# bergmanlab/TELR

Measured on AMD Instinct MI355X. Metric: gbp_aligned_per_s, higher is better.
Workload: dtype int16

## Files before the change

telr_amd/csrc/kernels.hip.h:

```cpp
#pragma once
#include <hip/hip_runtime.h>
#include <stdint.h>

#define TELR_NEG      (-(1 << 28))
#include "part_plan.h"
#define SK_TILE       1024
#define SK_THREADS    256
#define DP_DMAX       4096

struct ChainOpt {
    int32_t max_gap, bw, min_cnt, min_chain_score, chain_gap_q8, chain_skip_q8;
    int32_t dense_n, dense_span, mw_n;
};
struct DpOpt {
    int32_t a, b, q, e, q2, e2, sc_ambi, zdrop;
    int32_t cx_scale, cx_open, cx_emax, cx_emin, cx_dec, cx_flat;
};
__host__ __device__ __forceinline__ int d_cx_ext(const DpOpt &o, int len) { int v = o.cx_emax - o.cx_dec * len; return v > o.cx_emin ? v : o.cx_emin; }
__host__ __device__ __forceinline__ int d_cx_cost(const DpOpt &o, int L)
{
    int t = o.cx_open;
    for (int i = 0; i < L && i < o.cx_flat; ++i) t += d_cx_ext(o, i);
    if (L > o.cx_flat) t += (L - o.cx_flat) * o.cx_emin;
    return t;
// ... 3219 lines not shown
                const int delta = mx < -8192 ? 0 : mx;
                const uint32_t dd = pk_dup(delta), thr = pk_dup(delta - 12000);
#define REB_ONE(x) { const uint32_t dead = pk_sign(pk_sub((x), thr)); (x) = pk_sel(dead, PK_NEG, pk_max(pk_sub((x), dd), PK_NEG)); }
#pragma unroll
                for (int r = 0; r < R; ++r) { REB_ONE(He[r]) REB_ONE(Ho[r]) REB_ONE(E1e[r]) REB_ONE(E1o[r]) REB_ONE(F1e[r]) REB_ONE(F1o[r]) }
#undef REB_ONE
                off += delta;
            }
        }
        if (NW > 1) {
            if (wl == 63) { uint32_t *x = xch + (1 * NW + wv) * 3; x[0] = Ho[R - 1]; x[1] = E1o[R - 1]; x[2] = E2o[R - 1]; }
            __syncthreads();
        }
        if (EXT && __all(done)) break;
    }
    if (EXT) {
        if (have && l == 0) {
            DpRes Rr; Rr.score = best; Rr.bi = bi; Rr.bj = bj; Rr.nops = 0; Rr.mlen = 0; Rr.cells = ncell; Rr.tbases = n; Rr.mcols = 0;
            A.res[prob] = Rr;
        }
        return;
    }
    if (fin_here) {
        int sc = (int)(short)(fin_hi ? (fin >> 16) : (fin & 0xffffu)) + fin_off;
        if constexpr (TB4) sc >>= 2;
        if constexpr (TAG8) sc >>= 3;
        DpRes Rr; Rr.score = sc; Rr.bi = m; Rr.bj = n; Rr.nops = 0; Rr.mlen = 0; Rr.cells = P.pad[1]; Rr.tbases = n; Rr.mcols = 0;
        A.res[prob] = Rr;
    }
}

#define PK_NC 9
static_assert(__builtin_popcount(CLSM_PK) == PK_NC, "PK_NC counts the DPF_PK rows of DP_CLASS");
__host__ __device__ __forceinline__ constexpr int PK_IDX(int cls) { return __builtin_popcount(CLSM_PK & ((1u << cls) - 1u)); }
__host__ __device__ __forceinline__ constexpr int PK_CLS(int c) { int cls = 0; for (int k = 0; k < DP_NCLS; ++k) if (d_cls_in(k, CLSM_PK) && PK_IDX(k) == c) cls = k; return cls; }
struct PkPlan { int32_t woff[PK_NC + 1]; };
__global__ void k_pk_waves(const DpProb *__restrict__ probs, const int32_t *__restrict__ cls_list, ClsOff off, PkPlan plan,
                           uint32_t *__restrict__ keys, uint32_t *__restrict__ vals)
{
    const int i = blockIdx.x * blockDim.x + threadIdx.x;
    if (i >= plan.woff[PK_NC]) return;
    int c = 0;
    while (i >= plan.woff[c + 1]) ++c;
    const int cls = PK_CLS(c), first = (i - plan.woff[c]) * (64 / DP_CLASS[cls].lpp);
    const DpProb P = probs[cls_list[off.off[cls] + first]];
    const uint32_t cost = (uint32_t)((P.m + P.n) * DP_CLASS[cls].regs);
    keys[i] = cost > 0xFFFFu ? 0xFFFFu : cost;
    vals[i] = (uint32_t)cls << 26 | (uint32_t)first;
}
enum PkCell : int { CELL_PLAIN, CELL_TAG8, CELL_CX, CELL_ONEP, CELL_NIBBLE };
__device__ __forceinline__ int d_pk_cell(int cls, const DpOpt &o, int tb4, int tag8_steps, const DpProb *__restrict__ probs, const int32_t *__restrict__ first)
{
    if (o.cx_scale) return CELL_CX;
    const int onep_d = d_onep_d(o.q, o.e, o.q2, o.e2);
    static_assert(DP_CLASS[CLS_PK16].nibble == 1 && DP_CLASS[CLS_PK20].nibble == 2, "the nibble classes and their tb4_mask bits");
    if ((cls == CLS_PK16 && onep_d >= DP_CLASS[CLS_PK16].maxd) || (cls == CLS_PK20 && onep_d >= DP_CLASS[CLS_PK20].maxd)) return d_tb4(cls, tb4) ? CELL_NIBBLE : CELL_ONEP;
    const DpProb P0 = probs[*first];
    return P0.m + P0.n <= tag8_steps ? CELL_TAG8 : CELL_PLAIN;
}
template <int CLS, bool EXACT, bool ONEP, bool TB4, bool TAG8, bool CX>
__device__ __forceinline__ void d_dp_pk_cls(const DpArgs &A, const int32_t *__restrict__ list, int n, int first)
{
    static_assert(DP_CLASS[CLS].family == DPF_PK && EXACT == (DP_CLASS[CLS].layout == TBL_INTERLEAVED && CLS != CLS_PK16), "class table");
    d_dp_pkr<DP_CLASS[CLS].lpp, DP_CLASS[CLS].regs, false, 1, EXACT ? DP_CLASS[CLS].regs - 1 : 0, ONEP, TB4, TAG8, CX>(A, list, n, first);
}
template <bool TAG8, bool CX>
__device__ __forceinline__ void d_dp_pk_any(int cls, const DpArgs &A, const int32_t *__restrict__ list, int n, int first)
{
    switch (cls) {
    case CLS_PK20: d_dp_pk_cls<CLS_PK20, true, false, false, TAG8, CX>(A, list, n, first); break;
    case CLS_PK24: d_dp_pk_cls<CLS_PK24, true, false, false, TAG8, CX>(A, list, n, first); break;
    case CLS_PK28: d_dp_pk_cls<CLS_PK28, true, false, false, TAG8, CX>(A, list, n, first); break;
    case CLS_PK32: d_dp_pk_cls<CLS_PK32, true, false, false, TAG8, CX>(A, list, n, first); break;
    case CLS_PK16: d_dp_pk_cls<CLS_PK16, false, false, false, TAG8, CX>(A, list, n, first); break;
    case CLS_PK40: d_dp_pk_cls<CLS_PK40, false, false, false, TAG8, CX>(A, list, n, first); break;
    case CLS_PK48: d_dp_pk_cls<CLS_PK48, false, false, false, TAG8, CX>(A, list, n, first); break;
    case CLS_PK128: d_dp_pk_cls<CLS_PK128, false, false, false, TAG8, CX>(A, list, n, first); break;
    default: d_dp_pk_cls<CLS_PK64, false, false, false, TAG8, CX>(A, list, n, first); break;
    }
}
#ifndef PK_WPE
#define PK_WPE 2
#endif
__global__ void __launch_bounds__(64) __attribute__((amdgpu_waves_per_eu(PK_WPE))) k_dp_pk(DpArgs A, const uint32_t *__restrict__ waves, const int32_t *__restrict__ cls_list,
                                              ClsOff off)
{
    const uint32_t w = waves[blockIdx.x];
    const int cls = (int)(w >> 26), first = (int)(w & 0x3ffffffu);
    const int32_t *list = cls_list + off.off[cls];
    const int n = off.off[cls + 1] - off.off[cls];
    const int cell = d_pk_cell(cls, A.o, A.tb4, A.tag8_steps, A.probs, list + first);
    if (cell == CELL_CX) { d_dp_pk_any<false, true>(cls, A, list, n, first); return; }
    if (cell >= CELL_ONEP && cls == CLS_PK16) { if (cell == CELL_NIBBLE) d_dp_pk_cls<CLS_PK16, false, true, true, false, false>(A, list, n, first); else d_dp_pk_cls<CLS_PK16, false, true, false, false, false>(A, list, n, first); return; }
    if (cell >= CELL_ONEP) { if (cell == CELL_NIBBLE) d_dp_pk_cls<CLS_PK20, true, true, true, false, false>(A, list, n, first); else d_dp_pk_cls<CLS_PK20, true, true, false, false, false>(A, list, n, first); return; }
    if (cell == CELL_TAG8) { d_dp_pk_any<true, false>(cls, A, list, n, first); return; }
    d_dp_pk_any<false, false>(cls, A, list, n, first);
}
template <int NW>
__global__ void __launch_bounds__(64 * NW) k_dp_pkw(DpArgs A)
{
    __shared__ uint32_t xch[2 * NW * 3 + NW];
    __builtin_amdgcn_s_setprio(3);
    if (A.o.cx_scale) d_dp_pkr<64 * NW, 1, false, NW, 0, false, false, false, true>(A, A.list, A.nlist, blockIdx.x, xch);
    else d_dp_pkr<64 * NW, 1, false, NW>(A, A.list, A.nlist, blockIdx.x, xch);
}
constexpr int PKX_LPP = DP_CLASS[CLS_PKX64].lpp, PKX_R = DP_CLASS[CLS_PKX64].regs;
__global__ void __launch_bounds__(64) k_dp_pkx(DpArgs A)
{
    __builtin_amdgcn_s_setprio(3);
    if (A.o.cx_scale) d_dp_pkr<PKX_LPP, PKX_R, true, 1, 0, false, false, false, true>(A, A.list, A.nlist, blockIdx.x * (64 / PKX_LPP));
    else d_dp_pkr<PKX_LPP, PKX_R, true>(A, A.list, A.nlist, blockIdx.x * (64 / PKX_LPP));
}
__global__ void __launch_bounds__(64) k_dp_pkx16(DpArgs A)
{
    __builtin_amdgcn_s_setprio(3);
    if (A.o.cx_scale) d_dp_pkr<16, 1, true, 1, 0, false, false, false, true>(A, A.list, A.nlist, blockIdx.x * 4);
    else d_dp_pkr<16, 1, true>(A, A.list, A.nlist, blockIdx.x * 4);
}

constexpr int PKX8_LPP = DP_CLASS[CLS_PKX128].lpp;
static_assert(DP_CLASS[CLS_PKX128].regs == 32 / PKX8_LPP && DP_CLASS[CLS_PKX256].lpp == 16 && DP_CLASS[CLS_PKX256].regs == 4, "class table");
__global__ void __launch_bounds__(64) k_dp_pkx_w8(DpArgs A)
{
    __builtin_amdgcn_s_setprio(3);
    if (A.o.cx_scale) d_dp_pkr<PKX8_LPP, 32 / PKX8_LPP, true, 1, 0, false, false, false, true>(A, A.list, A.nlist, blockIdx.x * (64 / PKX8_LPP));
    else d_dp_pkr<PKX8_LPP, 32 / PKX8_LPP, true>(A, A.list, A.nlist, blockIdx.x * (64 / PKX8_LPP));
}
__global__ void __launch_bounds__(64) k_dp_pkx_w16(DpArgs A)
{
    __builtin_amdgcn_s_setprio(3);
    if (A.o.cx_scale) d_dp_pkr<16, 4, true, 1, 0, false, false, false, true>(A, A.list, A.nlist, blockIdx.x * 4);
    else d_dp_pkr<16, 4, true>(A, A.list, A.nlist, blockIdx.x * 4);
}

#ifndef TB_SLOTS
#define TB_SLOTS 2
#endif
template <int LAYOUT>
__device__ __forceinline__ void d_traceback_lane(const DpProb *__restrict__ probs, DpRes *__restrict__ res, int pi,
                                                 const uint8_t *__restrict__ tb_all, uint32_t *__restrict__ cig, int32_t *__restrict__ retry,
                                                 uint32_t *stage)
{
    const int lane = threadIdx.x;
    const DpProb P = probs[pi];
    if (P.kind >= 3) return;
    const int dhi_ = P.dhi; int touched = 0;
    const int cls = P.pad[0] & 0xff, dlo = P.dlo, mg = P.pad[0] >> 8;
    const int D = P.dhi - dlo + 1, stride = (D + 2) / 2;
    const int lpp = d_cls_slots(cls);
    const bool packed = d_tb_regs(cls), tiled = d_tb_tiled(cls), rows2 = d_tb_rows2(cls);
    int i = res[pi].bi, j = res[pi].bj;
    uint32_t *cg = cig + P.cig_off;
    int no = 0, ml = 0, mc = 0, state = 0, cur_op = -1, cur_len = 0;
    const int rowb = tiled ? lpp * 16 : packed ? lpp * 4 : stride;
    int64_t tag0 = -1, tag1 = -1, pfb = -2;
    uint4 v0 = make_uint4(0, 0, 0, 0), v1 = v0, v2 = v0, v3 = v0, v4 = v0, v5 = v0, v6 = v0, v7 = v0;
    while (i > 0 && j > 0) {
        const int a = i + j, sl = (j - i - dlo) >> 1;
        const int64_t off = tiled ? ((((int64_t)(a >> 3) * (4 * lpp) + ((sl >> 3) << 4) + (((a >> 1) & 3) << 2) + ((sl >> 1) & 3)) << 2) + ((a & 1) << 1) + (sl & 1))
                          : (LAYOUT == 2 || rows2) ? ((((int64_t)(a >> 1) * lpp + (sl >> 1)) << 2) + ((a & 1) << 1) + (sl & 1))
                          : packed ? ((((int64_t)(a >> 2) * lpp + sl) << 2) + (a & 3)) : ((int64_t)a * stride + sl);
        const int64_t abs_off = P.tb_off + (d_tb_interleaved(cls) ? ((off >> 3) << 9) + (off & 7) : off), line = abs_off >> 6;
        const int slot = TB_SLOTS > 1 ? (int)(line & 1) : 0;
        if ((slot ? tag1 : tag0) != line) {
            const int64_t blk = line >> 1;
            if (pfb != blk) {
                const uint4 *src = (const uint4*)(tb_all + (blk << 7));
                v0 = src[0]; v1 = src[1]; v2 = src[2]; v3 = src[3]; v4 = src[4]; v5 = src[5]; v6 = src[6]; v7 = src[7];
            }
            uint32_t *dst = stage + slot * 1024 + lane;
            if (line & 1) {
                dst[0 * 64] = v4.x; dst[1 * 64] = v4.y; dst[2 * 64] = v4.z; dst[3 * 64] = v4.w;
                dst[4 * 64] = v5.x; dst[5 * 64] = v5.y; dst[6 * 64] = v5.z; dst[7 * 64] = v5.w;
                dst[8 * 64] = v6.x; dst[9 * 64] = v6.y; dst[10 * 64] = v6.z; dst[11 * 64] = v6.w;
                dst[12 * 64] = v7.x; dst[13 * 64] = v7.y; dst[14 * 64] = v7.z; dst[15 * 64] = v7.w;
            } else {
                dst[0 * 64] = v0.x; dst[1 * 64] = v0.y; dst[2 * 64] = v0.z; dst[3 * 64] = v0.w;
                dst[4 * 64] = v1.x; dst[5 * 64] = v1.y; dst[6 * 64] = v1.z; dst[7 * 64] = v1.w;
                dst[8 * 64] = v2.x; dst[9 * 64] = v2.y; dst[10 * 64] = v2.z; dst[11 * 64] = v2.w;
                dst[12 * 64] = v3.x; dst[13 * 64] = v3.y; dst[14 * 64] = v3.z; dst[15 * 64] = v3.w;
            }
            if (slot) tag1 = line; else tag0 = line;
            const int64_t nl = rowb >= 64 ? (abs_off - rowb) >> 6 : line - 1, nb = nl >> 1;
            pfb = blk;
            if (nb != blk && nl >= 0) {
                const uint4 *src = (const uint4*)(tb_all + (nb << 7));
                v0 = src[0]; v1 = src[1]; v2 = src[2]; v3 = src[3]; v4 = src[4]; v5 = src[5]; v6 = src[6]; v7 = src[7];
                pfb = nb;
            }
        }
        const int w = (int)(abs_off & 63);
        const uint8_t *st8 = (const uint8_t*)stage + ((slot * 1024 + lane) << 2);
        const uint32_t t = st8[(w >> 2) * 256 + (w & 3)];
        const int mij = i < j ? i : j, kr = tiled ? (a >> 1) & 3 : 0;
        const bool up1 = kr >= 1 && mij > 1, up2 = kr >= 2 && mij > 2, up3 = kr >= 3 && mij > 3;
        const uint32_t t1 = up1 ? st8[((w - 16) >> 2) * 256 + (w & 3)] : 0xffu, t2 = up2 ? st8[((w - 32) >> 2) * 256 + (w & 3)] : 0xffu, t3 = up3 ? st8[((w - 48) >> 2) * 256 + (w & 3)] : 0xffu;
        const uint32_t nd = (uint32_t)((t1 & 7u) != 0u) << 1 | (uint32_t)((t2 & 7u) != 0u) << 2 | (uint32_t)((t3 & 7u) != 0u) << 3;
        const uint32_t mb = (t >> 7) | ((t1 >> 7) & 1u) << 1 | ((t2 >> 7) & 1u) << 2 | ((t3 >> 7) & 1u) << 3;
        touched |= (j - i - dlo <= mg) | (dhi_ - (j - i) <= mg);
        const int s0 = state ? state : (int)(t & 7);
        const int isM = s0 == 0, isD = s0 & 1;
        const int op = isM ? 0 : (isD ? 2 : 1);
        const int nn = isM ? __builtin_ctz(nd | 16u) : 1;
        state = (isM || !((t >> (2 + s0)) & 1)) ? 0 : s0;
        ml += isM ? __builtin_popcount(mb & ((1u << nn) - 1u)) : 0; mc += isM ? nn : 0;
        i -= isM ? nn : (isD ^ 1); j -= isM ? nn : isD;
        const bool same = op == cur_op;
        if (!same && cur_len) cg[no++] = (uint32_t)cur_len << 4 | (uint32_t)cur_op;
        cur_len = same ? cur_len + nn : nn; cur_op = op;
    }
    if (i > 0) { if (cur_op == 1) cur_len += i; else { if (cur_len) cg[no++] = (uint32_t)cur_len << 4 | (uint32_t)cur_op; cur_op = 1; cur_len = i; } }
    if (j > 0) { if (cur_op == 2) cur_len += j; else { if (cur_len) cg[no++] = (uint32_t)cur_len << 4 | (uint32_t)cur_op; cur_op = 2; cur_len = j; } }
    if (cur_len) cg[no++] = (uint32_t)cur_len << 4 | (uint32_t)cur_op;
    res[pi].nops = no; res[pi].mlen = ml; res[pi].mcols = mc;
    if (retry && P.kind == 0 && touched && P.m + P.n <= ADAPT_MAX_STEPS) retry[pi] = 1;
}
__global__ void __launch_bounds__(64) k_traceback(const DpProb *__restrict__ probs, DpRes *__restrict__ res, int32_t np,
                                                  const uint8_t *__restrict__ tb_all, uint32_t *__restrict__ cig, int32_t *__restrict__ retry,
                                                  const int32_t *__restrict__ list)
{
// ... 35 lines not shown
                x0 = make_uint4(u0.x, u0.y, u1.x, u1.y); x1 = make_uint4(u2.x, u2.y, u3.x, u3.y); x2 = make_uint4(u4.x, u4.y, u5.x, u5.y); x3 = make_uint4(u6.x, u6.y, u7.x, u7.y); } \
            else { const uint4 *src = (const uint4*)(tb + ((int64_t)L__ << 6)); x0 = src[0]; x1 = src[1]; x2 = src[2]; x3 = src[3]; } } } while (0)
#define TBR_PUT(dst_, x0, x1, x2, x3) do { uint32_t *dst = (dst_); \
            dst[0 * 64] = x0.x; dst[1 * 64] = x0.y; dst[2 * 64] = x0.z; dst[3 * 64] = x0.w; dst[4 * 64] = x1.x; dst[5 * 64] = x1.y; dst[6 * 64] = x1.z; dst[7 * 64] = x1.w; \
            dst[8 * 64] = x2.x; dst[9 * 64] = x2.y; dst[10 * 64] = x2.z; dst[11 * 64] = x2.w; dst[12 * 64] = x3.x; dst[13 * 64] = x3.y; dst[14 * 64] = x3.z; dst[15 * 64] = x3.w; } while (0)
#define TBR_ENSURE(L_) do { const int Le = (L_); \
            if (Le & 1) { if (tag1 != Le) { TBR_PUT(stage + 1024 + lane, b0, b1, b2, b3); tag1 = Le; TBR_FETCH(Le - 2, b0, b1, b2, b3); } } \
            else        { if (tag0 != Le) { TBR_PUT(stage + lane, a0, a1, a2, a3); tag0 = Le; TBR_FETCH(Le - 2, a0, a1, a2, a3); } } } while (0)
        if (ltop & 1) { TBR_FETCH(ltop, b0, b1, b2, b3); TBR_FETCH(ltop - 1, a0, a1, a2, a3); }
        else { TBR_FETCH(ltop, a0, a1, a2, a3); TBR_FETCH(ltop - 1, b0, b1, b2, b3); }
        for (int L = ltop; L >= 0; --L) {
            TBR_ENSURE(L);
            const int lim = L << 6;
            for (;;) {
                const int a = i + j, sl = (j - i - dlo) >> 1;
                const int o = nib ? (a >> 1) * rb4 + ((sl >> 2) << 2) + (((sl >> 1) & 1) << 1) + (sl & 1)
                                  : (((a >> 1) * lpp + (sl >> 1)) << 2) + ((a & 1) << 1) + (sl & 1);
                const bool act = i > 0 && j > 0 && o >= lim;
                if (!__any(act)) break;
                const int oo = act ? o : 0;
#define TBR_BYTE(x) ((uint32_t)stage8[((((x) >> 6) & 1) * 1024 + (((x) & 63) >> 2) * 64 + lane) * 4 + ((x) & 3)])
                const uint8_t *stage8 = (const uint8_t*)stage;
                uint32_t t = TBR_BYTE(oo);
                const int mij = i < j ? i : j, room = o - lim;
                const bool v1 = act && mij > 1 && room >= rowb, v2 = act && mij > 2 && room >= 2 * rowb, v3 = act && mij > 3 && room >= 3 * rowb;
                const uint32_t t1 = TBR_BYTE(v1 ? oo - rowb : 0), t2 = TBR_BYTE(v2 ? oo - 2 * rowb : 0), t3 = TBR_BYTE(v3 ? oo - 3 * rowb : 0);
#undef TBR_BYTE
                uint32_t nd, mb;
                if constexpr (ENC == 2) {
                    const int sh = (a & 1) << 2;
                    nd = (uint32_t)(!v1 || ((t1 >> sh) & 3u) != 2u) << 1 | (uint32_t)(!v2 || ((t2 >> sh) & 3u) != 2u) << 2 | (uint32_t)(!v3 || ((t3 >> sh) & 3u) != 2u) << 3;
                    mb = 0;
                    const uint32_t nb = (t >> sh) & 0xfu;
                    t = (2u - (nb & 3u)) | (nb & 4u) | ((nb & 8u) ^ 8u);
                } else if constexpr (ENC == 1) {
                    nd = (uint32_t)(!v1 || (t1 & 7u) != 4u) << 1 | (uint32_t)(!v2 || (t2 & 7u) != 4u) << 2 | (uint32_t)(!v3 || (t3 & 7u) != 4u) << 3;
                    mb = 0;
                    t = (4u - (t & 7u)) | (t & 0x28u) | ((t & 0x50u) ^ 0x50u);
                } else {
                    nd = (uint32_t)(!v1 || (t1 & 7u) != 0u) << 1 | (uint32_t)(!v2 || (t2 & 7u) != 0u) << 2 | (uint32_t)(!v3 || (t3 & 7u) != 0u) << 3;
                    mb = (t >> 7) | (t1 >> 7) << 1 | (t2 >> 7) << 2 | (t3 >> 7) << 3;
                }
                if (act) {
                    touched |= (j - i - dlo <= mg) | (dhi_ - (j - i) <= mg);
                    const int s0 = state ? state : (int)(t & (nib ? 3 : 7));
                    const int isM = s0 == 0, isD = s0 & 1;
                    const int op = isM ? 0 : (isD ? 2 : 1);
                    const int nn = isM ? __builtin_ctz(nd | 16u) : 1;
                    if (!isM) gc += (s0 <= 2 ? o_.e : o_.e2) + (state ? 0 : (s0 <= 2 ? o_.q : o_.q2));
                    state = (isM || !((t >> ((nib ? 1 : 2) + s0)) & 1)) ? 0 : s0;
                    ml += isM ? __builtin_popcount(mb & ((1u << nn) - 1u)) : 0; mc += isM ? nn : 0;
                    i -= isM ? nn : (isD ^ 1); j -= isM ? nn : isD;
                    const bool same = op == cur_op;
                    if (!same && cur_len) cg[no++] = (uint32_t)cur_len << 4 | (uint32_t)cur_op;
                    cur_len = same ? cur_len + nn : nn; cur_op = op;
                }
            }
            if (!__any(i > 0 && j > 0)) break;
        }
#undef TBR_FETCH
#undef TBR_PUT
#undef TBR_ENSURE
    }
    if (!have) return;
    if (i > 0) { const int c1 = o_.q + o_.e * i, c2 = o_.q2 + o_.e2 * i; gc += c1 < c2 ? c1 : c2; }
    if (j > 0) { const int c1 = o_.q + o_.e * j, c2 = o_.q2 + o_.e2 * j; gc += c1 < c2 ? c1 : c2; }
    if (i > 0) { if (cur_op == 1) cur_len += i; else { if (cur_len) cg[no++] = (uint32_t)cur_len << 4 | (uint32_t)cur_op; cur_op = 1; cur_len = i; } }
    if (j > 0) { if (cur_op == 2) cur_len += j; else { if (cur_len) cg[no++] = (uint32_t)cur_len << 4 | (uint32_t)cur_op; cur_op = 2; cur_len = j; } }
    if (cur_len) cg[no++] = (uint32_t)cur_len << 4 | (uint32_t)cur_op;
    if (nib || tag8) ml = (res[pi].score + o_.b * mc + gc) / (o_.a + o_.b);
    res[pi].nops = no; res[pi].mlen = ml; res[pi].mcols = mc;
    if (retry && P.kind == 0 && touched && P.m + P.n <= ADAPT_MAX_STEPS) retry[pi] = 1;
}
#ifdef TB_PROF
__device__ unsigned long long g_tb_prof[8];
#endif
__global__ void __launch_bounds__(64) k_traceback_pk(const DpProb *__restrict__ probs, DpRes *__restrict__ res,
                                                     const uint8_t *__restrict__ tb_all, uint32_t *__restrict__ cig, int32_t *__restrict__ retry,
                                                     const uint32_t *__restrict__ waves, const int32_t *__restrict__ cls_list, ClsOff off, int32_t tb4, DpOpt o, int32_t tag8_steps)
{
    __shared__ uint32_t stage[TB_SLOTS * 16 * 64];
    const uint32_t w = waves[blockIdx.x];
    const int cls = (int)(w >> 26), first = (int)(w & 0x3ffffffu);
    const int ppw = 64 / DP_CLASS[cls].lpp, t = threadIdx.x;
    const bool have = t < ppw && first + t < off.off[cls + 1] - off.off[cls];
    const int cell = d_pk_cell(cls, o, tb4, tag8_steps, probs, cls_list + off.off[cls] + first), rb4 = cell == CELL_NIBBLE ? d_tb4_rowb(cls) : 0;
    const bool tag8 = cell == CELL_TAG8;
#ifdef TB_PROF
    const unsigned long long t0_ = wall_clock64();
#endif
    const int pi_ = cls_list[off.off[cls] + (have ? first + t : first)], lpp_ = d_cls_slots(cls);
    if (d_tb_interleaved(cls)) {
        if (rb4) d_traceback_rows<2, true>(probs, res, pi_, have, lpp_, rb4, o, tb_all, cig, retry, stage);
        else if (tag8) d_traceback_rows<1, true>(probs, res, pi_, have, lpp_, 0, o, tb_all, cig, retry, stage);
        else d_traceback_rows<0, true>(probs, res, pi_, have, lpp_, 0, o, tb_all, cig, retry, stage);
    } else if (tag8) d_traceback_rows<1, false>(probs, res, pi_, have, lpp_, 0, o, tb_all, cig, retry, stage);
    else d_traceback_rows<0, false>(probs, res, pi_, have, lpp_, 0, o, tb_all, cig, retry, stage);
#ifdef TB_PROF
    if (threadIdx.x == 0) {
        const unsigned long long t1_ = wall_clock64(), dt = t1_ - t0_;
        const int rowb_ = rb4 ? rb4 : d_cls_slots(cls) * 4;
        const DpProb P0 = probs[cls_list[off.off[cls] + first]];
        unsigned long long lines = (unsigned long long)(((P0.m + P0.n) / 2 + 1) * rowb_ + 63) >> 6; if (lines > 65535) lines = 65535;
        atomicAdd(&g_tb_prof[0], dt); atomicMax(&g_tb_prof[1], dt << 16 | lines); atomicAdd(&g_tb_prof[2], 1ULL); atomicAdd(&g_tb_prof[3], lines);
        atomicMin(&g_tb_prof[4], t0_); atomicMax(&g_tb_prof[5], t1_);
    }
#endif
}

__global__ void __launch_bounds__(64) k_traceback_w(const DpProb *__restrict__ probs, DpRes *__restrict__ res, int32_t np,
                                                    const uint8_t *__restrict__ tb_all, uint32_t *__restrict__ cig, int32_t *__restrict__ retry,
                                                    const int32_t *__restrict__ list)
{
    __shared__ uint32_t win[64 * 16];
    const int lane = threadIdx.x;
    if ((int)blockIdx.x >= np) return;
    const int pi = list ? list[blockIdx.x] : (int)blockIdx.x;
    const DpProb P = probs[pi];
    if (P.kind >= 3) return;
    const int dhi_ = P.dhi; int touched = 0;
    const int cls = P.pad[0] & 0xff, dlo = P.dlo, mg = P.pad[0] >> 8;
    const int D = P.dhi - dlo + 1, stride = (D + 2) / 2;
    const int lpp = d_cls_slots(cls);
    const bool packed = d_tb_regs(cls), rows2 = d_tb_rows2(cls);
    const int64_t rowb = packed ? (int64_t)lpp * 4 : stride;
    const uint8_t *tb = tb_all + P.tb_off;
    int i = res[pi].bi, j = res[pi].bj;
    uint32_t *cg = cig + P.cig_off;
    int no = 0, ml = 0, mc = 0, state = 0, cur_op = -1, cur_len = 0;
    int r0 = -1; int64_t c0 = 0;
    while (i > 0 && j > 0) {
        const int a = i + j, sl = (j - i - dlo) >> 1;
        int row; int64_t col;
        if (rows2) { row = a >> 1; col = ((int64_t)(sl >> 1) << 2) + ((a & 1) << 1) + (sl & 1); }
        else if (packed) { row = a >> 2; col = ((int64_t)sl << 2) + (a & 3); }
        else { row = a; col = sl; }
        const int k = r0 - row;
        if (r0 < 0 || k < 0 || k >= 64 || col < c0 || col >= c0 + 64) {
            __syncthreads();
            r0 = row; c0 = col - 32; if (c0 < 0) c0 = 0; c0 &= ~3LL;
            const int rk = r0 - lane;
            uint32_t v[16];
#pragma unroll
            for (int x = 0; x < 16; ++x) v[x] = 0;
            if (rk >= 0) {
                const int64_t byte0 = (int64_t)rk * rowb + c0;
                const uint32_t *src = (const uint32_t*)(tb + (byte0 & ~3LL));
                const int sh = (int)(byte0 & 3) * 8;
                if (sh == 0) {
#pragma unroll
                    for (int x = 0; x < 16; ++x) v[x] = src[x];
                } else {
                    uint32_t prev = src[0];
#pragma unroll
                    for (int x = 0; x < 16; ++x) { const uint32_t nx = src[x + 1]; v[x] = (prev >> sh) | (nx << (32 - sh)); prev = nx; }
                }
            }
#pragma unroll
            for (int x = 0; x < 16; ++x) win[lane * 16 + x] = v[x];
            __syncthreads();
        }
        const int w = (int)(col - c0);
        touched |= (j - i - dlo <= mg) | (dhi_ - (j - i) <= mg);
        if (state == 0) {
            const int ik = i - lane, jk = j - lane, ak = a - 2 * lane;
            int rowk; int64_t colk;
            if (rows2) { rowk = ak >> 1; colk = ((int64_t)(sl >> 1) << 2) + ((ak & 1) << 1) + (sl & 1); }
            else if (packed) { rowk = ak >> 2; colk = ((int64_t)sl << 2) + (ak & 3); }
            else { rowk = ak; colk = sl; }
            const int kk = r0 - rowk, wk = (int)(colk - c0);
            const bool inw = ik > 0 && jk > 0 && kk < 64 && wk >= 0 && wk < 64;
            const uint32_t tk = inw ? (win[kk * 16 + (wk >> 2)] >> ((wk & 3) * 8)) & 0xffu : 0xffu;
            const uint64_t stop = ~__ballot(inw && (tk & 7u) == 0u);
            const int run = stop ? __builtin_ctzll(stop) : 64;
            if (run > 0) {
                const uint64_t low = run >= 64 ? ~0ULL : (1ULL << run) - 1;
                ml += __builtin_popcountll(__ballot(inw && (tk >> 7)) & low); mc += run; i -= run; j -= run;
                if (cur_op == 0) cur_len += run;
                else { if (cur_len && lane == 0) cg[no] = (uint32_t)cur_len << 4 | (uint32_t)cur_op; if (cur_len) ++no; cur_op = 0; cur_len = run; }
                continue;
// ... 203 lines not shown
```

telr_amd/csrc/telr_engine.hip:

```cpp
#include <hip/hip_runtime.h>
#include <cstring>
#include <string.h>
#include <rocprim/rocprim.hpp>
#include <algorithm>
#include <atomic>
#include <immintrin.h>
#include <chrono>
#include <cmath>
#include <condition_variable>
#include <cstdio>
#include <cstdlib>
#include <cstring>
#include <map>
#include <memory>
#include <mutex>
#include <string>
#include <thread>
#include <sys/mman.h>
#include <vector>
#include "../../include/telr_hip.h"
#include "kernels.hip.h"
#include "range_plan.h"
#include "sam_records.h"
#define TELR_HAVE_SEED_ARGS 1
// ... 1337 lines not shown
        HIPCHK(rocprim::radix_sort_pairs(tmp, tbytes, d_clskey, d_keytmp, d_listtmp, d_clslist, (size_t)np, 0, 24, st));
    }
    if (np > 0) {
        int64_t *d_tbs;
        TRY(ctx_buf_t(ctx, ("tb_sorted" + sfx).c_str(), (size_t)np + 1, &d_tbs));
        hipLaunchKernelGGL(k_tb_gather, dim3(np / 256 + 1), dim3(256), 0, st, d_tbb, d_clslist, np, coff, d_tbs);
        TRY((dev_exclusive_scan<int64_t, int64_t>(ctx, d_tbs, d_tboff, (size_t)np + 1)));
        hipLaunchKernelGGL(k_tb_scatter, dim3(np / 256 + 1), dim3(256), 0, st, d_probs, d_clslist, np, coff, d_tboff);
        HIPCHK(hipGetLastError());
        HIPCHK(hipMemcpyAsync(&tb_total, d_tboff + np, 8, hipMemcpyDeviceToHost, st));
        HIPCHK(hipStreamSynchronize(st));
    }
    uint8_t *d_tb;
    TRY(ctx_buf_t(ctx, ("tb" + sfx).c_str(), (size_t)tb_total + 256, &d_tb));
    if (primary) TRY(ctx_buf_t(ctx, "rawcig", (size_t)cg_total + 16, d_rawcig_io));
    DpArgs D; D.qseq2 = qs->d_seq2; D.qnmask = qs->d_nmask; D.tseq2 = tg->d_seq2; D.tnmask = tg->d_nmask; D.probs = d_probs;
    D.qtot = qs->padded_bases; D.ttot = tg->padded_bases;
    D.o.a = mo->a; D.o.b = mo->b; D.o.q = mo->q; D.o.e = mo->e; D.o.q2 = mo->q2; D.o.e2 = mo->e2; D.o.sc_ambi = mo->sc_ambi; D.o.zdrop = mo->zdrop;
    D.o.cx_scale = D.o.cx_open = D.o.cx_emax = D.o.cx_emin = D.o.cx_dec = D.o.cx_flat = 0;
    if (mo->cx_scale > 0) {
        const int S = mo->cx_scale;
        D.o.a *= S; D.o.b *= S; D.o.sc_ambi *= S; D.o.zdrop *= S;
        D.o.cx_scale = S; D.o.cx_open = mo->cx_open; D.o.cx_emax = mo->cx_ext_max; D.o.cx_emin = mo->cx_ext_min; D.o.cx_dec = mo->cx_decay;
        D.o.cx_flat = mo->cx_decay > 0 && mo->cx_ext_max > mo->cx_ext_min ? (mo->cx_ext_max - mo->cx_ext_min + mo->cx_decay - 1) / mo->cx_decay : 0;
    }
    D.tb = d_tb; D.cig = *d_rawcig_io; D.res = d_res; D.dcap = 0;
    D.retry = d_retry; D.tb4 = L.tb4_mask; D.tag8_steps = L.tag8_steps;
    static const bool tb_split = !ab_on("tb_one_launch");
    int nw = 0; uint32_t *d_wv2 = nullptr;
    {
        PkPlan plan; plan.woff[0] = 0;
        for (int c = 0; c < PK_NC; ++c) { const int ppw = 64 / DP_CLASS[PK_CLS(c)].lpp; plan.woff[c + 1] = plan.woff[c] + (h_cls[PK_CLS(c)] + ppw - 1) / ppw; }
        nw = plan.woff[PK_NC];
        if (nw > 0) {
            uint32_t *d_wk, *d_wv, *d_wk2;
            TRY(ctx_buf_t(ctx, ("pk_wkey" + sfx).c_str(), (size_t)nw, &d_wk));
            TRY(ctx_buf_t(ctx, ("pk_wval" + sfx).c_str(), (size_t)nw, &d_wv));
            TRY(ctx_buf_t(ctx, ("pk_wkey2" + sfx).c_str(), (size_t)nw, &d_wk2));
            TRY(ctx_buf_t(ctx, ("pk_wval2" + sfx).c_str(), (size_t)nw, &d_wv2));
            hipLaunchKernelGGL(k_pk_waves, dim3((nw + 255) / 256), dim3(256), 0, st, d_probs, d_clslist, coff, plan, d_wk, d_wv);
            HIPCHK(hipGetLastError());
            size_t tbytes = 0;
            HIPCHK(rocprim::radix_sort_pairs_desc(nullptr, tbytes, d_wk, d_wk2, d_wv, d_wv2, (size_t)nw, 0, 16, st));
            void *tmp; TRY(ctx_buf(ctx, "rp_tmp", tbytes, &tmp));
            HIPCHK(rocprim::radix_sort_pairs_desc(tmp, tbytes, d_wk, d_wk2, d_wv, d_wv2, (size_t)nw, 0, 16, st));
        }
    }
    HIPCHK(hipEventRecord(ctx->ev_fork, st));
    int side = 0;
    std::vector<hipStream_t> used;
    static const bool serial = getenv("TELR_SERIAL") != nullptr;
    auto side_stream = [&]() { if (serial) return st; hipStream_t s2 = ctx->side[side % TELR_NSIDE]; ++side; used.push_back(s2); return s2; };
    auto launch = [&](int c, DpKernel kernel, hipStream_t s2) -> int {
        const int nl = h_cls[c];
        int threads = DP_CLASS[c].lpp > 64 ? DP_CLASS[c].lpp : 64, ppb = DP_CLASS[c].lpp < 64 ? 64 / DP_CLASS[c].lpp : 1;
        size_t lds = 0;
        D.list = d_clslist + coff.off[c]; D.nlist = nl; D.dcap = 0;
        if (DP_CLASS[c].family == DPF_LDS) {
            D.dcap = DP_CLASS[c].maxd;
            lds = (size_t)(D.dcap + 2) * 5 * 4;
            static const bool one_wave = ab_on("dp_one_wave");
            if (one_wave) { kernel = k_dp; threads = 64; }
            if (lds > 48 * 1024) HIPCHK(hipFuncSetAttribute((const void*)kernel, hipFuncAttributeMaxDynamicSharedMemorySize, (int)lds));
        }
        if (c == CLS_PKX64 && nl < 8192) { kernel = k_dp_pkx16; ppb = 4; }
        hipLaunchKernelGGL(kernel, dim3((nl + ppb - 1) / ppb), dim3(threads), lds, s2, D);
        HIPCHK(hipGetLastError());
        return TELR_OK;
    };
    for (const SideLaunch &row : SIDE_LAUNCH) {
        const int c = row.cls, nl = h_cls[c];
        if (nl == 0) continue;
        hipStream_t s2 = side_stream();
        HIPCHK(hipStreamWaitEvent(s2, ctx->ev_fork, 0));
        TRY(launch(c, row.kernel, s2));
        if (tb_split) {
            const int tbw_max = 2048;
            if (row.lane_walk || nl > tbw_max) hipLaunchKernelGGL(k_traceback, dim3((nl + 63) / 64), dim3(64), 0, s2, d_probs, d_res, nl, d_tb, *d_rawcig_io, d_retry, D.list);
            else hipLaunchKernelGGL(k_traceback_w, dim3(nl), dim3(64), 0, s2, d_probs, d_res, nl, d_tb, *d_rawcig_io, d_retry, D.list);
            HIPCHK(hipGetLastError());
        }
    }
    D.dcap = 0;
    const bool tb_over = tb_split && !serial && nw > 0;
    if (primary) HIPCHK(hipEventRecord(ctx->evk[5], st));
    if (primary && nw > 0) ++ctx->pk_launches;
    if (nw > 0) {
        D.list = nullptr; D.nlist = 0;
        if (tb_over) { HIPCHK(hipStreamWaitEvent(ctx->tb_stream, ctx->ev_fork, 0)); if (primary) HIPCHK(hipEventRecord(ctx->evk[3], ctx->tb_stream)); }
        hipLaunchKernelGGL(k_dp_pk, dim3(nw), dim3(64), 0, st, D, d_wv2, d_clslist, coff);
        HIPCHK(hipGetLastError());
        if (tb_over) {
            HIPCHK(hipEventRecord(ctx->ev_pk, st));
            HIPCHK(hipStreamWaitEvent(ctx->tb_stream, ctx->ev_pk, 0));
            hipLaunchKernelGGL(k_traceback_pk, dim3(nw), dim3(64), 0, ctx->tb_stream, d_probs, d_res, d_tb, *d_rawcig_io, d_retry, d_wv2, d_clslist, coff, L.tb4_mask, D.o, L.tag8_steps);
            HIPCHK(hipGetLastError());
            if (primary) HIPCHK(hipEventRecord(ctx->evk[4], ctx->tb_stream));
            used.push_back(ctx->tb_stream);
        }
    }
    if (primary) HIPCHK(hipEventRecord(ctx->evk[0], st));
    if (h_cls[CLS_REG64]) TRY(launch(CLS_REG64, reg_kernel<CLS_REG64>(), st));
    if (h_cls[CLS_REG128]) TRY(launch(CLS_REG128, reg_kernel<CLS_REG128>(), st));
    if (primary) HIPCHK(hipEventRecord(ctx->evk[1], st));
    if (tb_split) {
        if (!tb_over && primary) HIPCHK(hipEventRecord(ctx->evk[3], st));
        if (!tb_over && nw > 0) hipLaunchKernelGGL(k_traceback_pk, dim3(nw), dim3(64), 0, st, d_probs, d_res, d_tb, *d_rawcig_io, d_retry, d_wv2, d_clslist, coff, L.tb4_mask, D.o, L.tag8_steps);
        for (int c : { (int)CLS_REG128, (int)CLS_REG64 }) {
            if (h_cls[c] == 0) continue;
            hipLaunchKernelGGL(k_traceback, dim3((h_cls[c] + 63) / 64), dim3(64), 0, st, d_probs, d_res, h_cls[c], d_tb, *d_rawcig_io, d_retry, (const int32_t*)(d_clslist + coff.off[c]));
        }
        if (!tb_over && primary) HIPCHK(hipEventRecord(ctx->evk[4], st));
        HIPCHK(hipGetLastError());
    }
    for (size_t u = 0; u < used.size(); ++u) {
        HIPCHK(hipEventRecord(ctx->ev_side[u % TELR_NSIDE], used[u]));
        HIPCHK(hipStreamWaitEvent(st, ctx->ev_side[u % TELR_NSIDE], 0));
    }
#ifdef TB_PROF
    if (nw > 0) {
        HIPCHK(hipDeviceSynchronize());
        unsigned long long h[8]; HIPCHK(hipMemcpyFromSymbol(h, HIP_SYMBOL(g_tb_prof), sizeof(h)));
        unsigned long long z[8] = {0, 0, 0, 0, ~0ULL, 0, 0, 0}; HIPCHK(hipMemcpyToSymbol(HIP_SYMBOL(g_tb_prof), z, sizeof(z)));
        if (h[2]) fprintf(stderr, "[tb prof] k_traceback_pk: %llu waves, span %.3f ms, longest wave %.3f ms (%llu lines), mean wave %.3f ms, %.1f lines per wave, wave-ms / span = %.1f waves on the device on average\n",
                          h[2], (double)(h[5] - h[4]) / 1e5, (double)(h[1] >> 16) / 1e5, h[1] & 0xffffULL, (double)h[0] / (double)h[2] / 1e5, (double)h[3] / (double)h[2], (double)h[0] / (double)(h[5] - h[4] ? h[5] - h[4] : 1));
    }
#endif
    if (!tb_split) {
        if (primary) HIPCHK(hipEventRecord(ctx->evk[3], st));
        hipLaunchKernelGGL(k_traceback, dim3((np + 63) / 64), dim3(64), 0, st, d_probs, d_res, np, d_tb, *d_rawcig_io, d_retry, (const int32_t*)nullptr);
        if (primary) HIPCHK(hipEventRecord(ctx->evk[4], st));
    }
    HIPCHK(hipGetLastError());
    return TELR_OK;
}

struct HostTrace {
    bool on; const char *tag; std::chrono::steady_clock::time_point t0, last;
    HostTrace(const char *t) : tag(t) { static const bool e = trace_on("host"); on = e; t0 = last = std::chrono::steady_clock::now(); }
    void mark(const char *what) {
        if (!on) return;
        auto now = std::chrono::steady_clock::now();
        fprintf(stderr, "[host %s] %-28s +%7.3f ms  (%8.3f)\n", tag, what, std::chrono::duration<double, std::milli>(now - last).count(), std::chrono::duration<double, std::milli>(now - t0).count());
        last = now;
    }
};

struct OccCut { int32_t mid_occ; const int32_t *d_tmid; };
static int chain_dispatch(telr_ctx *ctx, hipStream_t st, const telr_map_opt *mo, const uint64_t *d_skeys, const int32_t *d_qaoff, int nq, int32_t na,
                          int32_t n_over, const int32_t *d_overlist, const int32_t *d_qorder, int32_t *d_f, int32_t *d_p)
{
    ChainOpt co; co.max_gap = mo->max_gap; co.bw = mo->bw_long > mo->bw ? mo->bw_long : mo->bw; co.min_cnt = mo->min_cnt; co.min_chain_score = mo->min_chain_score;
    co.chain_gap_q8 = mo->chain_gap_q8; co.chain_skip_q8 = mo->chain_skip_q8;
    static const bool chain_push = ab_on("chain_push"), chain_lazy = ab_on("chain_lazy"), chain_no_mw = ab_on("chain_no_mw");
    static int dense_v[3] = {2048, 48, 1 << 19};
    static const bool dense_env = [] { if (const char *e = getenv("TELR_CHAIN_DENSE")) sscanf(e, "%d%*[,:]%d%*[,:]%d", &dense_v[0], &dense_v[1], &dense_v[2]); return true; }();
    (void)dense_env;
    const int Rr = mo->chain_lookback / 64;
    const bool mw_all = dense_v[2] <= SEGSORT_CAP;
    static const bool no_islands = ab_on("no_islands");
    static const bool chain_no_pack = ab_on("chain_no_pack");
    const bool islands = nq <= CHAIN_ISL_NQ && na > 0 && !no_islands;
    const bool mw = !(mo->flags & TELR_MF_CHAIN_SKIP) && !chain_push && !chain_lazy && !chain_no_mw && Rr >= 2 && na > 0 && !islands && dense_v[2] > 0 && (mw_all || n_over > 0);
    co.dense_n = dense_v[0]; co.dense_span = dense_v[1]; co.mw_n = mw ? dense_v[2] : 0;
#define CHAIN_LAUNCH(RR, SK) do { if (chain_push) hipLaunchKernelGGL((k_chain<RR, SK, 0>), dim3(nq), dim3(64), 0, st, d_skeys, d_qaoff, nq, co, d_f, d_p, d_qorder, 0, 0); \
                                  else if (chain_lazy) hipLaunchKernelGGL((k_chain<RR, SK, 1>), dim3(nq), dim3(64), 0, st, d_skeys, d_qaoff, nq, co, d_f, d_p, d_qorder, 0, 0); \
                                  else hipLaunchKernelGGL((k_chain<RR, SK, 2>), dim3(nq), dim3(64), 0, st, d_skeys, d_qaoff, nq, co, d_f, d_p, d_qorder, mw ? 1 : 0, chain_no_pack ? 0 : 1); } while (0)
#define CHAIN_MW(RR, SK) hipLaunchKernelGGL((k_chain_mw<RR, SK>), dim3(mw_all ? nq : n_over), dim3(64 * RR), 0, ctx->side[0], d_skeys, d_qaoff, mw_all ? nq : n_over, mw_all ? (const int32_t*)nullptr : (const int32_t*)d_overlist, co, d_f, d_p)
    const bool skip = co.chain_skip_q8 != 0;
    if (mo->flags & TELR_MF_CHAIN_SKIP) {
        int32_t *d_mark;
        TRY(ctx_buf_t(ctx, "chain_mark", (size_t)na + 1, &d_mark));
        if (islands) {
            int32_t *d_head, *d_rank, *d_ioff, *d_ipd;
            TRY(ctx_buf_t(ctx, "isl_head", (size_t)na + 1, &d_head));
            TRY(ctx_buf_t(ctx, "isl_rank", (size_t)na + 1, &d_rank));
            TRY(ctx_buf_t(ctx, "isl_off", (size_t)na + 2, &d_ioff));
            TRY(ctx_buf_t(ctx, "isl_pd", (size_t)na + 1, &d_ipd));
            HIPCHK(hipMemsetAsync(d_head + na, 0, 4, st));
            hipLaunchKernelGGL(k_isl_heads, dim3(nq), dim3(256), 0, st, d_skeys, d_qaoff, nq, (uint32_t)co.max_gap, d_head);
            HIPCHK(hipGetLastError());
            TRY((dev_exclusive_scan<int32_t, int32_t>(ctx, d_head, d_rank, (size_t)na + 1)));
            hipLaunchKernelGGL(k_isl_fill, dim3(nq), dim3(256), 0, st, d_qaoff, nq, d_head, d_rank, (int32_t)na, d_ioff, d_ipd);
            const unsigned grid = (unsigned)std::min<int64_t>((int64_t)na, 256 * 32);
            if (skip) hipLaunchKernelGGL(k_chain_scan_isl<true>, dim3(grid), dim3(64), 0, st, d_skeys, d_ioff, d_ipd, d_rank + na, co, d_f, d_p, d_mark);
            else hipLaunchKernelGGL(k_chain_scan_isl<false>, dim3(grid), dim3(64), 0, st, d_skeys, d_ioff, d_ipd, d_rank + na, co, d_f, d_p, d_mark);
        } else if (nq > 0) {
            if (skip) hipLaunchKernelGGL(k_chain_scan<true>, dim3(nq), dim3(64), 0, st, d_skeys, d_qaoff, nq, co, d_f, d_p, d_mark, d_qorder);
            else hipLaunchKernelGGL(k_chain_scan<false>, dim3(nq), dim3(64), 0, st, d_skeys, d_qaoff, nq, co, d_f, d_p, d_mark, d_qorder);
        }
// ... 1447 lines not shown
```

Measured before the change: 23.53.

## Fuse packed-class traceback into the k_dp_pk DP kernel

Adds a WALK template flag to k_dp_pk so each wave runs the traceback for its own problems right after the DP fill, replacing the separate k_traceback_pk launch by default. An ab flag keeps the old split path. The aim is to drop a kernel launch and the cross-stream event wait, and to read traceback data while it may still be in cache. In exchange the DP kernel now reserves shared staging memory and needs more registers, which can lower occupancy. It also gives up the overlap of traceback with the REG-class kernels on the separate traceback stream.

```diff
diff --git a/telr_amd/csrc/kernels.hip.h b/telr_amd/csrc/kernels.hip.h
--- a/telr_amd/csrc/kernels.hip.h
+++ b/telr_amd/csrc/kernels.hip.h
@@ -3325,6 +3325,30 @@
 #ifndef PK_WPE
 #define PK_WPE 2
 #endif
+#ifndef TB_SLOTS
+#define TB_SLOTS 2
+#endif
+template <int ENC, bool IL>
+__device__ __forceinline__ void d_traceback_rows(const DpProb *__restrict__ probs, DpRes *__restrict__ res, int pi, bool have, int lpp, int rb4_, const DpOpt o_,
+                                                 const uint8_t *__restrict__ tb_all, uint32_t *__restrict__ cig, int32_t *__restrict__ retry,
+                                                 uint32_t *stage);
+__device__ __forceinline__ void d_traceback_pk_wave(int cls, int first, int cell, const DpProb *__restrict__ probs, DpRes *__restrict__ res,
+                                                    const uint8_t *__restrict__ tb_all, uint32_t *__restrict__ cig, int32_t *__restrict__ retry,
+                                                    const int32_t *__restrict__ cls_list, const ClsOff &off, const DpOpt &o, uint32_t *stage)
+{
+    const int ppw = 64 / DP_CLASS[cls].lpp, t = threadIdx.x;
+    const bool have = t < ppw && first + t < off.off[cls + 1] - off.off[cls];
+    const int rb4 = cell == CELL_NIBBLE ? d_tb4_rowb(cls) : 0;
+    const bool tag8 = cell == CELL_TAG8;
+    const int pi_ = cls_list[off.off[cls] + (have ? first + t : first)], lpp_ = d_cls_slots(cls);
+    if (d_tb_interleaved(cls)) {
+        if (rb4) d_traceback_rows<2, true>(probs, res, pi_, have, lpp_, rb4, o, tb_all, cig, retry, stage);
+        else if (tag8) d_traceback_rows<1, true>(probs, res, pi_, have, lpp_, 0, o, tb_all, cig, retry, stage);
+        else d_traceback_rows<0, true>(probs, res, pi_, have, lpp_, 0, o, tb_all, cig, retry, stage);
+    } else if (tag8) d_traceback_rows<1, false>(probs, res, pi_, have, lpp_, 0, o, tb_all, cig, retry, stage);
+    else d_traceback_rows<0, false>(probs, res, pi_, have, lpp_, 0, o, tb_all, cig, retry, stage);
+}
+template <bool WALK>
 __global__ void __launch_bounds__(64) __attribute__((amdgpu_waves_per_eu(PK_WPE))) k_dp_pk(DpArgs A, const uint32_t *__restrict__ waves, const int32_t *__restrict__ cls_list,
                                               ClsOff off)
 {
@@ -3333,11 +3357,16 @@
     const int32_t *list = cls_list + off.off[cls];
     const int n = off.off[cls + 1] - off.off[cls];
     const int cell = d_pk_cell(cls, A.o, A.tb4, A.tag8_steps, A.probs, list + first);
-    if (cell == CELL_CX) { d_dp_pk_any<false, true>(cls, A, list, n, first); return; }
-    if (cell >= CELL_ONEP && cls == CLS_PK16) { if (cell == CELL_NIBBLE) d_dp_pk_cls<CLS_PK16, false, true, true, false, false>(A, list, n, first); else d_dp_pk_cls<CLS_PK16, false, true, false, false, false>(A, list, n, first); return; }
-    if (cell >= CELL_ONEP) { if (cell == CELL_NIBBLE) d_dp_pk_cls<CLS_PK20, true, true, true, false, false>(A, list, n, first); else d_dp_pk_cls<CLS_PK20, true, true, false, false, false>(A, list, n, first); return; }
-    if (cell == CELL_TAG8) { d_dp_pk_any<true, false>(cls, A, list, n, first); return; }
-    d_dp_pk_any<false, false>(cls, A, list, n, first);
+    if (cell == CELL_CX) d_dp_pk_any<false, true>(cls, A, list, n, first);
+    else if (cell >= CELL_ONEP && cls == CLS_PK16) { if (cell == CELL_NIBBLE) d_dp_pk_cls<CLS_PK16, false, true, true, false, false>(A, list, n, first); else d_dp_pk_cls<CLS_PK16, false, true, false, false, false>(A, list, n, first); }
+    else if (cell >= CELL_ONEP) { if (cell == CELL_NIBBLE) d_dp_pk_cls<CLS_PK20, true, true, true, false, false>(A, list, n, first); else d_dp_pk_cls<CLS_PK20, true, true, false, false, false>(A, list, n, first); }
+    else if (cell == CELL_TAG8) d_dp_pk_any<true, false>(cls, A, list, n, first);
+    else d_dp_pk_any<false, false>(cls, A, list, n, first);
+    if constexpr (WALK) {
+        __shared__ uint32_t stage[TB_SLOTS * 16 * 64];
+        d_wave_sync();
+        d_traceback_pk_wave(cls, first, cell, A.probs, A.res, A.tb, A.cig, A.retry, cls_list, off, A.o, stage);
+    }
 }
 template <int NW>
 __global__ void __launch_bounds__(64 * NW) k_dp_pkw(DpArgs A)
@@ -3376,9 +3405,6 @@
     else d_dp_pkr<16, 4, true>(A, A.list, A.nlist, blockIdx.x * 4);
 }
 
-#ifndef TB_SLOTS
-#define TB_SLOTS 2
-#endif
 template <int LAYOUT>
 __device__ __forceinline__ void d_traceback_lane(const DpProb *__restrict__ probs, DpRes *__restrict__ res, int pi,
                                                  const uint8_t *__restrict__ tb_all, uint32_t *__restrict__ cig, int32_t *__restrict__ retry,
@@ -3580,20 +3606,12 @@
     __shared__ uint32_t stage[TB_SLOTS * 16 * 64];
     const uint32_t w = waves[blockIdx.x];
     const int cls = (int)(w >> 26), first = (int)(w & 0x3ffffffu);
-    const int ppw = 64 / DP_CLASS[cls].lpp, t = threadIdx.x;
-    const bool have = t < ppw && first + t < off.off[cls + 1] - off.off[cls];
-    const int cell = d_pk_cell(cls, o, tb4, tag8_steps, probs, cls_list + off.off[cls] + first), rb4 = cell == CELL_NIBBLE ? d_tb4_rowb(cls) : 0;
-    const bool tag8 = cell == CELL_TAG8;
+    const int cell = d_pk_cell(cls, o, tb4, tag8_steps, probs, cls_list + off.off[cls] + first);
 #ifdef TB_PROF
     const unsigned long long t0_ = wall_clock64();
+    const int rb4 = cell == CELL_NIBBLE ? d_tb4_rowb(cls) : 0;
 #endif
-    const int pi_ = cls_list[off.off[cls] + (have ? first + t : first)], lpp_ = d_cls_slots(cls);
-    if (d_tb_interleaved(cls)) {
-        if (rb4) d_traceback_rows<2, true>(probs, res, pi_, have, lpp_, rb4, o, tb_all, cig, retry, stage);
-        else if (tag8) d_traceback_rows<1, true>(probs, res, pi_, have, lpp_, 0, o, tb_all, cig, retry, stage);
-        else d_traceback_rows<0, true>(probs, res, pi_, have, lpp_, 0, o, tb_all, cig, retry, stage);
-    } else if (tag8) d_traceback_rows<1, false>(probs, res, pi_, have, lpp_, 0, o, tb_all, cig, retry, stage);
-    else d_traceback_rows<0, false>(probs, res, pi_, have, lpp_, 0, o, tb_all, cig, retry, stage);
+    d_traceback_pk_wave(cls, first, cell, probs, res, tb_all, cig, retry, cls_list, off, o, stage);
 #ifdef TB_PROF
     if (threadIdx.x == 0) {
         const unsigned long long t1_ = wall_clock64(), dt = t1_ - t0_;
diff --git a/telr_amd/csrc/telr_engine.hip b/telr_amd/csrc/telr_engine.hip
--- a/telr_amd/csrc/telr_engine.hip
+++ b/telr_amd/csrc/telr_engine.hip
@@ -1443,13 +1443,16 @@
         }
     }
     D.dcap = 0;
-    const bool tb_over = tb_split && !serial && nw > 0;
+    static const bool pk_split = ab_on("tb_pk_split");
+    const bool pk_fused = tb_split && !pk_split;
+    const bool tb_over = tb_split && !pk_fused && !serial && nw > 0;
     if (primary) HIPCHK(hipEventRecord(ctx->evk[5], st));
     if (primary && nw > 0) ++ctx->pk_launches;
     if (nw > 0) {
         D.list = nullptr; D.nlist = 0;
         if (tb_over) { HIPCHK(hipStreamWaitEvent(ctx->tb_stream, ctx->ev_fork, 0)); if (primary) HIPCHK(hipEventRecord(ctx->evk[3], ctx->tb_stream)); }
-        hipLaunchKernelGGL(k_dp_pk, dim3(nw), dim3(64), 0, st, D, d_wv2, d_clslist, coff);
+        if (pk_fused) hipLaunchKernelGGL(k_dp_pk<true>, dim3(nw), dim3(64), 0, st, D, d_wv2, d_clslist, coff);
+        else hipLaunchKernelGGL(k_dp_pk<false>, dim3(nw), dim3(64), 0, st, D, d_wv2, d_clslist, coff);
         HIPCHK(hipGetLastError());
         if (tb_over) {
             HIPCHK(hipEventRecord(ctx->ev_pk, st));
@@ -1466,7 +1469,7 @@
     if (primary) HIPCHK(hipEventRecord(ctx->evk[1], st));
     if (tb_split) {
         if (!tb_over && primary) HIPCHK(hipEventRecord(ctx->evk[3], st));
-        if (!tb_over && nw > 0) hipLaunchKernelGGL(k_traceback_pk, dim3(nw), dim3(64), 0, st, d_probs, d_res, d_tb, *d_rawcig_io, d_retry, d_wv2, d_clslist, coff, L.tb4_mask, D.o, L.tag8_steps);
+        if (!tb_over && !pk_fused && nw > 0) hipLaunchKernelGGL(k_traceback_pk, dim3(nw), dim3(64), 0, st, d_probs, d_res, d_tb, *d_rawcig_io, d_retry, d_wv2, d_clslist, coff, L.tb4_mask, D.o, L.tag8_steps);
         for (int c : { (int)CLS_REG128, (int)CLS_REG64 }) {
             if (h_cls[c] == 0) continue;
             hipLaunchKernelGGL(k_traceback, dim3((h_cls[c] + 63) / 64), dim3(64), 0, st, d_probs, d_res, h_cls[c], d_tb, *d_rawcig_io, d_retry, (const int32_t*)(d_clslist + coff.off[c]));
```

Result: no change. 23.64 (median of 4 runs) (+0.4%).
